# killerwhile/kafka-assignment-optimizer

Hardware: AMD Instinct MI355X
Metric: candidate assignments/sec (+ time_to_optimal_s), 10k-partition reassign (higher is better)
Workload: dtype int32

## Files before the change

### include/kao.h

```cpp
#ifndef KAO_H
#define KAO_H

#include <stdint.h>

#ifdef __cplusplus
extern "C" {
#endif

#define KAO_VERSION 103
#define KAO_NONE 0xFFFFu
#define KAO_MAX_RF 8
#define KAO_MAX_RACKS 255

enum {
    KAO_OK = 0,
    KAO_ERR_INVALID = -1,
    KAO_ERR_UNSUPPORTED = -2,
    KAO_ERR_NO_DEVICE = -3,
    KAO_ERR_HIP = -4,
    KAO_ERR_NOMEM = -5,
    KAO_ERR_NOT_INIT = -6
};

enum {
// ... 89 lines not shown
int kao_eval_plan_create(const kao_topic *t, kao_eval_plan **out);
int kao_eval_plan_run(kao_eval_plan *p, const void *d_candidates, int64_t n, void *d_objective ,
                      void *d_violations , void *d_best_key );
int kao_eval_plan_sync(kao_eval_plan *p, double *ms_last );
void kao_eval_plan_destroy(kao_eval_plan *p);

int kao_session_create(const kao_topic *topics, int32_t n_topics, const kao_opts *opts, kao_session **out);
int kao_session_step(kao_session *s);
int kao_session_sync(kao_session *s);
int kao_session_new_generation(kao_session *s);
int kao_session_best(kao_session *s, kao_result *results);
int kao_session_best_keys(kao_session *s, uint64_t *keys);
int kao_session_device_keys(kao_session *s, void **d_keys);
int kao_session_stats(kao_session *s, kao_stats *out);
int kao_session_small_launches(kao_session *s, int64_t *out);
int kao_session_chunked_launches(kao_session *s, int64_t *out);
int kao_search_chunk_plan(int32_t entries, int32_t resident, int32_t iters, int32_t forced, int32_t *out, int32_t cap);
int kao_session_bound_step(kao_session *s, const int64_t *target, int32_t iters);
int kao_session_set_prices(kao_session *s, int32_t topic, const int32_t *a, const int32_t *l, const int32_t *g);
int kao_session_adopt_prices(kao_session *s);
int kao_session_prices(kao_session *s, int32_t topic, int32_t *a, int32_t *l, int32_t *g);
int kao_session_bound_busy(kao_session *s);
int kao_session_bounds(kao_session *s, int64_t *upper_bound, int32_t *flags, int32_t *iters);
int kao_session_dual_state(kao_session *s, int32_t topic, int32_t *a, int32_t *l, int32_t *g, int64_t *best_dual);
int kao_session_set_dual_state(kao_session *s, int32_t topic, const int32_t *a, const int32_t *l, const int32_t *g);
int kao_lp_bound(const kao_topic *t, double tol, int32_t max_iters, int64_t *bound, int64_t *best_dual, int32_t *multipliers, double stats[8]);
int kao_lp_trace(const kao_topic *t, double tol, int32_t max_iters, double *trace, double stats[8], int32_t *multipliers);
int kao_lp_round(const kao_topic *t, double pert, uint32_t salt, double tol, int32_t max_iters, int32_t use_fallback, uint16_t *assignment,
                 int64_t *objective, int32_t violations[8], double stats[8]);
int kao_lp_round_host(const kao_topic *t, const uint8_t *q, const int32_t *zq, int32_t use_fallback, uint16_t *assignment, int32_t rep[4]);
int kao_dense_spd_test(const double *A, int32_t n, const double *rhs, double *factor, double *linv, double *x, double ms[2]);
int kao_search_band_row(int32_t lo, int32_t hi, int32_t c, int32_t force_plain, int32_t *fits);
int kao_search_rack_delta(int32_t lo, int32_t hi, int32_t c, int32_t dec);
int kao_lp_sharded_test(const kao_topic *t, const int32_t *devices, int32_t n_dev, double pert, uint32_t salt, double tol, int32_t max_iters,
                        int64_t *bound, uint16_t *assignment, int64_t *objective, int32_t violations[8], double stats[8]);
int kao_dual_bound(const kao_topic *t, int64_t target, int32_t iters, int32_t launches, int64_t *bound,
                   int64_t *best_dual, int32_t *iters_done, int32_t *flags, int32_t *multipliers);
int kao_session_restart_state(kao_session *s, int32_t topic, int32_t restart, uint16_t *final_state,
                              uint16_t *best_state, int32_t info[4]);
void kao_session_destroy(kao_session *s);

int kao_solve(const kao_topic *topics, int32_t n_topics, const kao_opts *opts, kao_result *results);
int kao_solve_multi(const kao_topic *topics, int32_t n_topics, const int32_t *devices, int32_t n_dev, const kao_opts *opts,
                    kao_result *results);
int kao_solve_capped(const kao_topic *topics, int32_t n_topics, const int32_t *replica_cap, const int32_t *devices, int32_t n_dev,
                     const kao_opts *opts, int32_t max_rounds, kao_result *results, int64_t *lagrangian_bound);
int kao_improve_cycles(const kao_topic *t, uint16_t *assignment, int32_t max_rounds, int64_t *objective, int32_t stats[8]);
int kao_cycle_matrices(const kao_topic *t, const uint16_t *assignment, int32_t layer, int32_t level, int32_t *dist, int32_t *mid,
                       uint32_t *slot);
int kao_cycle_square_plan(int32_t n, int32_t out[3]);
int kao_cycle_seeds(const kao_topic *t, const uint16_t *assignment, int32_t *table, int32_t *n_cfg);
int kao_cycle_pair_edges(const kao_topic *t, const uint16_t *assignment, int32_t gmin, int32_t *cost, int64_t stats[4]);

int kao_plan_waves(int32_t n_brokers, int32_t n_partitions, int32_t width, const uint16_t *current, const uint16_t *target,
                   int32_t max_per_broker, uint64_t seed, int32_t *wave , int32_t *n_waves, int32_t *lower_bound);

int kao_plan_waves_sized(int32_t n_brokers, int32_t n_partitions, int32_t width, const uint16_t *current, const uint16_t *target,
                         const uint64_t *size , uint64_t max_bytes_per_broker, int32_t max_per_broker,
                         uint64_t seed, int32_t *wave , int32_t *n_waves, int32_t *lower_bound);

int kao_balance_leaders(const kao_topic *t, uint16_t *assignment , int32_t *n_changed,
                        int64_t *objective ,
                        int32_t *status, int32_t stats[8] );

#define KAO_FAILOVER_MAX_BROKERS 8000
int kao_failover_order(int32_t n_brokers, int32_t n_racks, const uint8_t *rack_of ,
// ... 86 lines not shown
```

### kafka_assignment_optimizer_amd/_ffi.py

```python
from __future__ import annotations

import ctypes as C
import os

_HERE = os.path.dirname(os.path.abspath(__file__))
LIB_PATH = os.path.join(_HERE, "libkao.so")


class KaoTopic(C.Structure):
    _fields_ = [("n_brokers", C.c_int32), ("n_racks", C.c_int32), ("n_partitions", C.c_int32),
                ("rf", C.c_int32), ("rf_cur", C.c_int32),
                ("rack_of", C.POINTER(C.c_uint8)), ("current", C.POINTER(C.c_uint16)),
                ("w", (C.c_int32 * 2) * 2),
                ("rep_lo", C.c_int32), ("rep_hi", C.c_int32), ("lead_lo", C.c_int32), ("lead_hi", C.c_int32),
                ("rack_lo", C.c_int32), ("rack_hi", C.c_int32), ("prack_lo", C.c_int32), ("prack_hi", C.c_int32),
                ("broker_w", C.POINTER(C.c_int32)), ("broker_wl", C.POINTER(C.c_int32))]


class KaoOpts(C.Structure):
    _fields_ = [("seed", C.c_uint64), ("time_limit_s", C.c_double), ("restarts", C.c_int32),
                ("iters_per_launch", C.c_int32), ("max_launches", C.c_int32), ("obj_scale", C.c_int32),
                ("lam_min", C.c_int32), ("lam_max", C.c_int32), ("period_log2", C.c_int32),
                ("stop_at_bound", C.c_int32), ("profile", C.c_int32), ("dual_iters", C.c_int32),
                ("elite_period", C.c_int32), ("use_prices", C.c_int32), ("use_cycles", C.c_int32), ("islands", C.c_int32),
# ... 30 lines not shown
    "kao_evaluate": (C.c_int, [_P(KaoTopic), _P(C.c_uint16), _P(C.c_int64), _P(C.c_int32)]),
    "kao_evaluate_batch": (C.c_int, [_P(KaoTopic), _P(C.c_uint16), C.c_int64, _P(C.c_int32), _P(C.c_int32)]),
    "kao_eval_plan_create": (C.c_int, [_P(KaoTopic), _P(C.c_void_p)]),
    "kao_eval_plan_run": (C.c_int, [C.c_void_p, C.c_void_p, C.c_int64, C.c_void_p, C.c_void_p, C.c_void_p]),
    "kao_eval_plan_sync": (C.c_int, [C.c_void_p, _P(C.c_double)]),
    "kao_eval_plan_destroy": (None, [C.c_void_p]),
    "kao_session_create": (C.c_int, [_P(KaoTopic), C.c_int32, _P(KaoOpts), _P(C.c_void_p)]),
    "kao_session_step": (C.c_int, [C.c_void_p]),
    "kao_session_sync": (C.c_int, [C.c_void_p]),
    "kao_session_new_generation": (C.c_int, [C.c_void_p]),
    "kao_session_best": (C.c_int, [C.c_void_p, _P(KaoResult)]),
    "kao_session_best_keys": (C.c_int, [C.c_void_p, _P(C.c_uint64)]),
    "kao_session_device_keys": (C.c_int, [C.c_void_p, _P(C.c_void_p)]),
    "kao_session_stats": (C.c_int, [C.c_void_p, _P(KaoStats)]),
    "kao_session_small_launches": (C.c_int, [C.c_void_p, _P(C.c_int64)]),
    "kao_session_chunked_launches": (C.c_int, [C.c_void_p, _P(C.c_int64)]),
    "kao_search_chunk_plan": (C.c_int, [C.c_int32, C.c_int32, C.c_int32, C.c_int32, _P(C.c_int32), C.c_int32]),
    "kao_session_restart_state": (C.c_int, [C.c_void_p, C.c_int32, C.c_int32, _P(C.c_uint16), _P(C.c_uint16),
                                            _P(C.c_int32)]),
    "kao_session_bound_step": (C.c_int, [C.c_void_p, _P(C.c_int64), C.c_int32]),
    "kao_session_set_prices": (C.c_int, [C.c_void_p, C.c_int32, _P(C.c_int32), _P(C.c_int32), _P(C.c_int32)]),
    "kao_session_adopt_prices": (C.c_int, [C.c_void_p]),
    "kao_session_prices": (C.c_int, [C.c_void_p, C.c_int32, _P(C.c_int32), _P(C.c_int32), _P(C.c_int32)]),
    "kao_session_bound_busy": (C.c_int, [C.c_void_p]),
    "kao_session_bounds": (C.c_int, [C.c_void_p, _P(C.c_int64), _P(C.c_int32), _P(C.c_int32)]),
    "kao_session_dual_state": (C.c_int, [C.c_void_p, C.c_int32, _P(C.c_int32), _P(C.c_int32), _P(C.c_int32), _P(C.c_int64)]),
    "kao_session_set_dual_state": (C.c_int, [C.c_void_p, C.c_int32, _P(C.c_int32), _P(C.c_int32), _P(C.c_int32)]),
    "kao_lp_bound": (C.c_int, [_P(KaoTopic), C.c_double, C.c_int32, _P(C.c_int64), _P(C.c_int64), _P(C.c_int32), _P(C.c_double)]),
    "kao_lp_round": (C.c_int, [_P(KaoTopic), C.c_double, C.c_uint32, C.c_double, C.c_int32, C.c_int32, _P(C.c_uint16), _P(C.c_int64), _P(C.c_int32), _P(C.c_double)]),
    "kao_lp_round_host": (C.c_int, [_P(KaoTopic), _P(C.c_uint8), _P(C.c_int32), C.c_int32, _P(C.c_uint16), _P(C.c_int32)]),
    "kao_dense_spd_test": (C.c_int, [_P(C.c_double), C.c_int32, _P(C.c_double), _P(C.c_double), _P(C.c_double), _P(C.c_double), _P(C.c_double)]),
    "kao_search_band_row": (C.c_int, [C.c_int32, C.c_int32, C.c_int32, C.c_int32, _P(C.c_int32)]),
    "kao_search_rack_delta": (C.c_int, [C.c_int32, C.c_int32, C.c_int32, C.c_int32]),
    "kao_lp_sharded_test": (C.c_int, [_P(KaoTopic), _P(C.c_int32), C.c_int32, C.c_double, C.c_uint32, C.c_double, C.c_int32, _P(C.c_int64), _P(C.c_uint16),
                                      _P(C.c_int64), _P(C.c_int32), _P(C.c_double)]),
    "kao_lp_trace": (C.c_int, [_P(KaoTopic), C.c_double, C.c_int32, _P(C.c_double), _P(C.c_double), _P(C.c_int32)]),
    "kao_dual_bound": (C.c_int, [_P(KaoTopic), C.c_int64, C.c_int32, C.c_int32, _P(C.c_int64), _P(C.c_int64), _P(C.c_int32),
                                 _P(C.c_int32), _P(C.c_int32)]),
    "kao_session_destroy": (None, [C.c_void_p]),
    "kao_solve": (C.c_int, [_P(KaoTopic), C.c_int32, _P(KaoOpts), _P(KaoResult)]),
    "kao_solve_multi": (C.c_int, [_P(KaoTopic), C.c_int32, _P(C.c_int32), C.c_int32, _P(KaoOpts), _P(KaoResult)]),
    "kao_solve_capped": (C.c_int, [_P(KaoTopic), C.c_int32, _P(C.c_int32), _P(C.c_int32), C.c_int32, _P(KaoOpts), C.c_int32,
                                  _P(KaoResult), _P(C.c_int64)]),
    "kao_rccl_selftest": (C.c_int, [_P(C.c_int32), C.c_int32]),
    "kao_rccl_loopback_counts": (C.c_int, [_P(C.c_uint64)]),
    "kao_improve_cycles": (C.c_int, [_P(KaoTopic), _P(C.c_uint16), C.c_int32, _P(C.c_int64), _P(C.c_int32)]),
    "kao_cycle_matrices": (C.c_int, [_P(KaoTopic), _P(C.c_uint16), C.c_int32, C.c_int32, _P(C.c_int32), _P(C.c_int32), _P(C.c_uint32)]),
    "kao_cycle_square_plan": (C.c_int, [C.c_int32, _P(C.c_int32)]),
    "kao_cycle_seeds": (C.c_int, [_P(KaoTopic), _P(C.c_uint16), _P(C.c_int32), _P(C.c_int32)]),
    "kao_cycle_pair_edges": (C.c_int, [_P(KaoTopic), _P(C.c_uint16), C.c_int32, _P(C.c_int32), _P(C.c_int64)]),
    "kao_plan_waves": (C.c_int, [C.c_int32, C.c_int32, C.c_int32, _P(C.c_uint16), _P(C.c_uint16), C.c_int32, C.c_uint64,
                                 _P(C.c_int32), _P(C.c_int32), _P(C.c_int32)]),
    "kao_plan_waves_sized": (C.c_int, [C.c_int32, C.c_int32, C.c_int32, _P(C.c_uint16), _P(C.c_uint16), _P(C.c_uint64), C.c_uint64,
                                       C.c_int32, C.c_uint64, _P(C.c_int32), _P(C.c_int32), _P(C.c_int32)]),
    "kao_balance_leaders": (C.c_int, [_P(KaoTopic), _P(C.c_uint16), _P(C.c_int32), _P(C.c_int64), _P(C.c_int32), _P(C.c_int32)]),
    "kao_failover_order": (C.c_int, [C.c_int32, C.c_int32, _P(C.c_uint8), C.c_int32, C.c_int32, _P(C.c_uint16), C.c_int32, C.c_int32,
                                     _P(C.c_int32), _P(C.c_int32), _P(C.c_int32)]),
    "kao_balance_leaders_cluster": (C.c_int, [C.c_int32, C.c_int32, C.c_int32, _P(C.c_uint16), _P(C.c_int32), C.c_int32, _P(C.c_int32),
                                              _P(C.c_int32), C.c_int32, C.c_int32, C.c_int32, _P(C.c_int32), _P(C.c_int32), _P(C.c_int32),
                                              _P(C.c_int32), _P(C.c_int32)]),
    "kao_balance_leaders_weighted": (C.c_int, [C.c_int32, C.c_int32, C.c_int32, _P(C.c_uint16), _P(C.c_uint64), C.c_uint64, C.c_int32, C.c_int32,
                                               _P(C.c_int32), _P(C.c_uint64), _P(C.c_uint64), _P(C.c_uint64), _P(C.c_int32), _P(C.c_int64)]),
    "kao_wleaders_test_path": (C.c_int, [C.c_int32]),
    "kao_failover_order_weighted": (C.c_int, [C.c_int32, C.c_int32, _P(C.c_uint8), C.c_int32, C.c_int32, _P(C.c_uint16), _P(C.c_uint64), C.c_int32,
                                              C.c_uint64, C.c_int32, C.c_int32, _P(C.c_uint64), _P(C.c_int32), _P(C.c_int32), _P(C.c_int64)]),
    "kao_balance_disk": (C.c_int, [C.c_int32, C.c_int32, _P(C.c_uint8), C.c_int32, C.c_int32, _P(C.c_uint16), _P(C.c_uint64), C.c_int32, C.c_int32,
# ... 42 lines not shown
```

### kafka_assignment_optimizer_amd/csrc/kao_search.hip

```cpp
#include "kao_search_dev.h"

#include <map>
#include <mutex>
#include <tuple>

namespace kao {

struct SearchPiece {
    uint32_t entry;
    int32_t init, elite;
    uint32_t first, n;
    bool later;
    uint32_t ticket;
};
__device__ __forceinline__ void chunk_pass(uint32_t ticket);
template <class T> __device__ __forceinline__ T late_kernarg(size_t off) {
    auto p = (const __attribute__((address_space(4))) unsigned char *)__builtin_amdgcn_kernarg_segment_ptr();
    asm volatile("" : "+s"(p));
    return *reinterpret_cast<const __attribute__((address_space(4))) T *>(p + off);
}
static_assert(sizeof(SearchPools) % alignof(SearchParams) == 0, "late_kernarg: SearchParams follows SearchPools without padding");
constexpr size_t kArgPrm = sizeof(SearchPools);
__device__ __forceinline__ int4 sched_record(const int4 *sched, uint32_t ticket) {
    auto p = (const __attribute__((address_space(4))) int *)sched + 4 * (size_t)ticket;
// ... 193 lines not shown
        if (pc.later) rng = pl.chunk_rng[(size_t)g * 64 + lane];
        pl.chunk_rng[(size_t)g * 64 + lane] = pc.ticket;
    }

    const int plog = TD->period_log2 + (rho & 3);
    const uint32_t pmask = (1u << plog) - 1u;
    const uint32_t lrange = (uint32_t)(prm.lam_max - prm.lam_min + 1);
    const uint32_t RF8 = (uint32_t)T.RF << 8, R8 = (uint32_t)T.R << 8, m8 = (uint32_t)T.m << 8;

    const int T_tour = min(64, max(4, (T.P * T.RF) >> 2));
    uint32_t tour_off = lane < T_tour ? 0u : kKeyNull;
    asm volatile("" : "+v"(tour_off));
    const int GA = min(16, max(1, (T.P * T.RF) >> 8));
    const int x_rounds_full = (T.P + 63) >> 6;
    const bool x_windowed = x_rounds_full > 8;

    int lam_lo = prm.lam_min, lam_hi = prm.lam_max;
    uint32_t n_iters = kChunked ? pc.n : prm.iters, it_base = prm.launch * prm.iters + (kChunked ? pc.first : 0u);
    constexpr uint32_t kLpScanTwo = 1u << 29;
    uint32_t loop_pack = TD->P * TD->RF <= prm.scan2_max ? kLpScanTwo : 0u;
    if (kSmall) loop_pack |= ((uint32_t)prm.lam_min & 0xFFFu) | (((uint32_t)prm.lam_max & 0xFFFu) << 12) | (((uint32_t)plog & 31u) << 24);
    {
        uint32_t v0 = (uint32_t)lam_lo, v1 = (uint32_t)lam_hi, v2 = n_iters, v3 = it_base, v4 = loop_pack;
        asm volatile("" : "+v"(v2), "+v"(v3), "+v"(v4));
        if constexpr (!kSmall) {
            asm volatile("" : "+v"(v0), "+v"(v1));
            lam_lo = (int)__builtin_amdgcn_readfirstlane(v0); lam_hi = (int)__builtin_amdgcn_readfirstlane(v1);
        }
        n_iters = __builtin_amdgcn_readfirstlane(v2); it_base = __builtin_amdgcn_readfirstlane(v3);
        loop_pack = __builtin_amdgcn_readfirstlane(v4);
    }
    auto loop_flag = [&](uint32_t bit) { uint32_t lp = loop_pack; asm volatile("" : "+s"(lp)); return (lp & bit) != 0u; };
    constexpr bool kFuse = !kGlobalA && !kTeam && !kPriced;
    const bool fuse_ok = kFuse && T.Bx <= 16384;
    uint32_t jmp_a = 1u, jmp_c = 0u;
    if (fuse_ok)
        for (int n = (T.Bx + 63) >> 6; n > 0; --n) { jmp_a = (jmp_a * 0x6D2B79u) & 0xFFFFFFu; jmp_c = (jmp_c * 0x6D2B79u + 0x3C6EF3u) & 0xFFFFFFu; }
    best_obj = __builtin_amdgcn_readfirstlane(best_obj);
    for (uint32_t i = 0; i < n_iters; ++i) {
        const uint32_t it = it_base + i;
        const int type = (int)((0x1210u >> ((it & 7u) * 2u)) & 3u);
        int lam;
        if constexpr (kSmall) {
            uint32_t lp = loop_pack;
            asm volatile("" : "+s"(lp));
            const uint32_t plg = (lp >> 24) & 31u;
            const int lo_ = (int)(lp & 0xFFFu), hi_ = (int)((lp >> 12) & 0xFFFu);
            const uint32_t ph = it & ((1u << plg) - 1u);
            lam = best_obj < 0 ? hi_ : min(hi_, lo_ + (int)((2u * ph * (uint32_t)(hi_ - lo_ + 1)) >> plg));
        } else {
            const uint32_t ph = it & pmask;
            lam = best_obj < 0 ? lam_hi : min(lam_hi, lam_lo + (int)((2u * ph * lrange) >> plog));
        }
        const bool sampled = (type == 2) || (type == 0 && ((it >> 3) & 1u));

        auto finish = [&](auto ty, auto uni, uint32_t kmin, int win, int p, int k, int q, int j, uint32_t uw, uint32_t vw, int dV, int dObj) {
            constexpr int TY = decltype(ty)::value;
            auto of_win = [&](int v) { return decltype(uni)::value ? v : __builtin_amdgcn_readlane(v, win); };
            if (!kTeam) {
                if (kmin == kKeyNull) return;
                if ((int)(kmin >> 8) - kDBias > 0) return;
            }
            bool mine = true;
            int *rec = TR + ((i & 1u) * 16 + (uint32_t)wave) * kTeamRec;
            if (kTeam) {
                const bool ok = kmin != kKeyNull && (int)(kmin >> 8) - kDBias <= 0;
                if (lane == win) {
                    const uint32_t ro_ = uw >> 16, rn_ = vw >> 16;
                    const bool racks = ok && TY == 0 && ro_ != rn_;
                    rec[0] = ok ? 1 : 0; rec[1] = p; rec[2] = TY == 1 ? q : p;
                    rec[3] = (int)(uw & 0xFFFFu); rec[4] = (int)(vw & 0xFFFFu);
                    rec[5] = racks ? (int)ro_ : 0xFFFF; rec[6] = racks ? (int)rn_ : 0xFFFF;
                    rec[7] = dV; rec[8] = dObj;
                }
                __syncthreads();
                bool clash = false;
                if (lane < wave) {
                    const int *o = TR + ((i & 1u) * 16 + (uint32_t)lane) * kTeamRec;
                    if (o[0]) {
                        const int mp = rec[1], mq = rec[2], mb0 = rec[3], mb1 = rec[4], mr0 = rec[5], mr1 = rec[6];
                        clash = (o[1] == mp) | (o[1] == mq) | (o[2] == mp) | (o[2] == mq) | (o[3] == mb0) | (o[3] == mb1) | (o[4] == mb0) | (o[4] == mb1);
                        if (o[5] != 0xFFFF && mr0 != 0xFFFF) clash |= (o[5] == mr0) | (o[5] == mr1) | (o[6] == mr0) | (o[6] == mr1);
                    }
                }
                mine = ok && __ballot(clash) == 0ull;
            }

            constexpr bool kOneTrip = !kTeam && kSmall;
// ... 89 lines not shown
                        L.W[xx] = (uint16_t)wx;
                    }
                }
            }
            }
            if (kGlobalA) __builtin_amdgcn_fence(__ATOMIC_SEQ_CST, "workgroup");
            if (kTeam) {
                if (lane == 0) rec[9] = mine ? 1 : 0;
                __syncthreads();
                int dVs = 0, dOs = 0, na = 0;
                if (lane < n_waves) {
                    const int *o = TR + ((i & 1u) * 16 + (uint32_t)lane) * kTeamRec;
                    if (o[9]) { dVs = o[7]; dOs = o[8]; na = 1; }
                }
                V += wave_sum(dVs);
                obj += wave_sum(dOs);
                accepted += wave_sum(na);
            } else {
                V += of_win(dV);
                obj += of_win(dObj);
                accepted++;
            }
        };
        constexpr std::integral_constant<int, 0> kReplace{};
        constexpr std::integral_constant<int, 1> kExchange{};
        constexpr std::integral_constant<int, 2> kLeaderSwap{};

        if (sampled) {
            const int p = (int)rnd24_wide(rng, (uint32_t)T.P);
            const Part<NW> a = L.A[p];
            const Part<NW> c = CUR[p];
            uint32_t key = kKeyNull, vw = 0;
            int dV = 0, dObj = 0;
            if (type == 0) {
                const int k = (int)rnd24(rng, RF8);
                const uint32_t uw = sel_slot<NS>(a, k);
                const uint32_t ro = uw >> 16;
                const bool lead = k == 0;
                const uint32_t lw = lead ? 2u : 0u;
                const int wl = lead ? T.w00 : T.w01, wf = lead ? T.w10 : T.w11;
                const int g_old = role_w2<NS>(c, uw, wl, wf) + (hbw ? bw_of(BW[uw & 0xFFFFu], lead) : 0);
                const uint32_t wo = L.W[uw & 0xFFFFu];
                const int dV_old = wfld(wo, kWDecR) + wfldw(wo, kWDecL, lw);
                const int dV_rack_old = ddec(L.K[ro], T.rack_lo, T.rack_hi) + c7_delta(T.c7_dec, cnt4x2<NS>(a, ro));
                const int rsz_ro = RSZ[ro];
                int dP_old = 0, dP_rack_old = 0;
                if (kPriced) {
                    const uint32_t pro = PR[uw & 0xFFFFu];
                    dP_old = -(wflag(wo, kWPoutR) & price_rep(pro));
                    if (lead) dP_old -= wflag(wo, kWPoutL) & price_lead(pro);
                    dP_rack_old = p_out(L.K[ro], T.rack_lo, T.rack_hi, PG[ro]);
                }
                const int base_s = kSmall ? mad24s(S, g_old, kDBias) : 0;
#pragma unroll
                for (int g = 0; g < 4; ++g) {
                    uint32_t r, jj;
                    bool okg;
                    if (g < 2) {
                        r = rnd24(rng, R8);
                        jj = rnd24(rng, m8);
                        okg = (int)jj < RSZ[r];
                    } else {
                        r = ro;
                        jj = rnd24(rng, (uint32_t)rsz_ro << 8);
                        okg = true;
                    }
                    const uint32_t x = __umul24(r, (uint32_t)T.m) + jj;
// ... 162 lines not shown
#pragma unroll
                for (int s2 = 0; s2 < 2; ++s2) {
                    const int wA = s2 == 0 ? wA1 : wA2;
                    ps[s2] = __builtin_amdgcn_readlane(pl_, wA);
                    ks[s2] = __builtin_amdgcn_readlane(kl_, wA);
                    us[s2] = (uint32_t)__builtin_amdgcn_readlane((int)oldw_l, wA);
                    gs[s2] = __builtin_amdgcn_readlane(g_old_l, wA);
                    dvos[s2] = __builtin_amdgcn_readlane(dvo_l, wA);
                    v_rk[s2] = __builtin_amdgcn_readlane(dvr_l, wA);
                }
                const Part<NW> a1 = L.A[ps[0]], c1 = CUR[ps[0]], a2 = L.A[ps[1]], c2 = CUR[ps[1]];
                const uint32_t ro1 = us[0] >> 16, ro2 = us[1] >> 16;
                for (int r = lane; r < T.R; r += 64) {
                    const int dk = dinc(L.K[r], T.rack_lo, T.rack_hi);
                    const int v1 = ((uint32_t)r != ro1) ? v_rk[0] + dk + c7_delta(T.c7_inc, cnt4x2<NS>(a1, (uint32_t)r)) : 0;
                    const int v2 = ((uint32_t)r != ro2) ? v_rk[1] + dk + c7_delta(T.c7_inc, cnt4x2<NS>(a2, (uint32_t)r)) : 0;
                    L.RT[r] = kSmall ? (int)(((uint32_t)v2 & 0xFFFFu) | ((uint32_t)v1 << 16)) : (int)(((uint32_t)v1 & 0xFFFFu) | ((uint32_t)v2 << 16));
                }
                int lane_v = lane;
                asm volatile("" : "+v"(lane_v));
                const int li = lane_v & (NW - 1);
                const bool l2 = lane_v >= NW;
                const int p_l = l2 ? ps[1] : ps[0];
                const uint32_t ai = reinterpret_cast<const uint32_t *>(&L.A[p_l])[li], ci = reinterpret_cast<const uint32_t *>(&CUR[p_l])[li];
                const bool holds = (lane_v < 2 * NW) & (ai != kNoneW);
                uint32_t w_keep = 0;
                if (holds) w_keep = L.W[ai & 0xFFFFu];
                if (holds & !l2) L.W[ai & 0xFFFFu] = (uint16_t)(w_keep | kWNoCand);
                if (holds & l2) L.W[ai & 0xFFFFu] = (uint16_t)(L.W[ai & 0xFFFFu] | kWNoCand2);
                const bool hc = (lane_v < 2 * NW) & (ci != kNoneW);
                uint32_t w_ci = 0;
                if (hc) w_ci = L.W[ci & 0xFFFFu];
                const bool hm_l = hc & ((w_ci & (l2 ? kWNoCand2 : kWNoCand)) == 0u);
                const int mr_l = hm_l ? (int)((ci & 0xFFFFu) >> 6) : -1;
                int mr[2 * NW];
#pragma unroll
                for (int i2 = 0; i2 < 2 * NW; ++i2) mr[i2] = (i2 & (NW - 1)) < NS ? __builtin_amdgcn_readlane(mr_l, i2) : -1;
                const bool lead1 = ks[0] == 0, lead2 = ks[1] == 0;
                const uint32_t lw1 = lead1 ? 2u : 0u, lw2 = lead2 ? 2u : 0u;
                const int wl1 = lead1 ? T.w00 : T.w01, wf1 = lead1 ? T.w10 : T.w11, wl2 = lead2 ? T.w00 : T.w01, wf2 = lead2 ? T.w10 : T.w11;
                const int K01 = __mul24(S, gs[0]) + kDBias + __mul24(lam, dvos[0]);
                const int K02 = __mul24(S, gs[1]) + kDBias + __mul24(lam, dvos[1]);
                const uint32_t leadp = (lead2 ? 1u : 0u) | (lead1 ? 0x10000u : 0u);
                const uint32_t K0p = ((uint32_t)K02 & 0xFFFFu) | ((uint32_t)K01 << 16);
                const int wl1h = (int)((uint32_t)(S * wl1) << 16), wf1h = (int)((uint32_t)(S * wf1) << 16);
                const int wl2s = (int)((uint32_t)(S * wl2) & 0xFFFFu), wf2s = (int)((uint32_t)(S * wf2) & 0xFFFFu);
                uint32_t jc = jmp_c;
                asm volatile("" : "+v"(jc));
                uint32_t best1 = kKeyNull, best2 = kKeyNull;
                const short *Ws = reinterpret_cast<const short *>(L.W);
                auto scan_round2 = [&](auto with_w, int base, int rd, int w, int rt, uint32_t &key1, uint32_t &key2) {
                    const uint32_t st1 = lcg24(rng);
                    uint32_t st2;
                    asm("v_mad_u32_u24 %0, %1, %2, %3" : "=v"(st2) : "v"(st1), "s"(jmp_a), "v"(jc));
                    const int inc = wfld(w, kWIncR);
                    if constexpr (kSmall) {
                        uint32_t d = pk_mad_ss(pk_add(pk_mad_lo((uint32_t)wfld(w, kWIncL), leadp, (uint32_t)inc), (uint32_t)rt), (uint32_t)lam, K0p);
                        if (decltype(with_w)::value) {
                            const uint32_t x = (uint32_t)(base + lane);
                            const uint32_t xw = x | ((uint32_t)XR[x] << 16);
                            auto mask_of = [](bool b) { uint32_t m = b ? ~0u : 0u; asm("" : "+v"(m)); return m; };
                            const bool l1 = c1.w[0] == xw, l2 = c2.w[0] == xw;
                            bool f1 = false, f2 = false;
#pragma unroll
                            for (int i2 = 1; i2 < NS; ++i2) { f1 |= c1.w[i2] == xw; f2 |= c2.w[i2] == xw; }
                            auto and_or = [](uint32_t m, uint32_t w, uint32_t acc) { uint32_t r; asm("v_and_or_b32 %0, %1, %2, %3" : "=v"(r) : "v"(m), "s"(w), "v"(acc)); return r; };
                            uint32_t ws = mask_of(l1) & (uint32_t)wl1h;
                            ws = and_or(mask_of(f1), (uint32_t)wf1h, ws);
                            ws = and_or(mask_of(l2), (uint32_t)wl2s, ws);
                            ws = and_or(mask_of(f2), (uint32_t)wf2s, ws);
                            d = pk_sub(d, ws);
                        }
                        key1 = ((d | (uint32_t)w) & 0xFFFF0000u) | (st1 & 0xFF00u) | (uint32_t)rd;
                        key2 = ((d | (uint32_t)wflag(w, 14)) << 16) | (st2 & 0xFF00u) | (uint32_t)rd;
                        return;
                    }
                    int d1 = __mul24(lam, inc + wfldw(w, kWIncL, lw1) + wfldw(rt, 0, 16u)) + K01;
                    int d2 = __mul24(lam, inc + wfldw(w, kWIncL, lw2) + (rt >> 16)) + K02;
                    if (decltype(with_w)::value) {
                        const uint32_t x = (uint32_t)(base + lane);
                        const uint32_t xw = x | ((uint32_t)XR[x] << 16);
                        d1 -= __mul24(S, role_w2<NS>(c1, xw, wl1, wf1));
                        d2 -= __mul24(S, role_w2<NS>(c2, xw, wl2, wf2));
                    }
                    d1 = min(max(d1, 0), 2 * kDBias - 2);
                    d2 = min(max(d2, 0), 2 * kDBias - 2) | wflag(w, 14);
                    key1 = ((uint32_t)d1 << 16) | (st1 & 0xFF00u) | (uint32_t)rd | ((uint32_t)w & 0xFFFF0000u);
                    key2 = ((uint32_t)d2 << 16) | (st2 & 0xFF00u) | (uint32_t)rd;
                };
                const int n_rd = (T.Bx + 63) >> 6;
                int rd = 0, base = 0;
                while (rd < n_rd) {
                    int nxt = n_rd;
#pragma unroll
                    for (int i2 = 0; i2 < 2 * NW; ++i2)
                        if (mr[i2] >= rd) nxt = min(nxt, mr[i2]);
                    uint32_t k1a, k2a, k1b, k2b;
                    for (; rd + 1 < nxt; rd += 2, base += 128) {
                        const int wa = Ws[base + lane], wb = Ws[base + 64 + lane];
                        const uint32_t ra = XR[base + lane], rb = XR[base + 64 + lane];
                        const int rta = L.RT[ra], rtb = L.RT[rb];
                        scan_round2(std::false_type{}, base, rd, wa, rta, k1a, k2a);
                        scan_round2(std::false_type{}, base + 64, rd + 1, wb, rtb, k1b, k2b);
                        best1 = min(best1, min(k1a, k1b));
                        best2 = min(best2, min(k2a, k2b));
                    }
                    if (rd < nxt) { const int wa = Ws[base + lane]; scan_round2(std::false_type{}, base, rd, wa, L.RT[XR[base + lane]], k1a, k2a); best1 = min(best1, k1a); best2 = min(best2, k2a); ++rd; base += 64; }
                    if (rd < n_rd) { const int wa = Ws[base + lane]; scan_round2(std::true_type{}, base, rd, wa, L.RT[XR[base + lane]], k1a, k2a); best1 = min(best1, k1a); best2 = min(best2, k2a); ++rd; base += 64; }
                }
                asm("v_mad_u32_u24 %0, %0, %1, %2" : "+v"(rng) : "s"(jmp_a), "v"(jc));
                if (holds) L.W[ai & 0xFFFFu] = (uint16_t)w_keep;
                const uint32_t kw = wave_umin(min(((best1 >> 1) & ~127u) | (uint32_t)lane, ((best2 >> 1) & ~127u) | 64u | (uint32_t)lane));
                const bool two = (kw & 64u) != 0u;
                const uint32_t kmin = kw >> 7;
                const int win = (int)(kw & 63u);
                const int p = two ? ps[1] : ps[0], k = two ? ks[1] : ks[0];
                const uint32_t uw = two ? us[1] : us[0];
                if ((int)(kmin >> 8) - kDBias <= 0) {
                    const bool lead = k == 0;
                    const uint32_t bw_ = (uint32_t)__builtin_amdgcn_readlane((int)(two ? best2 : best1), win);
                    const uint32_t xs = ((bw_ & 255u) << 6) + (uint32_t)win;
                    const uint32_t rs = XR[xs];
                    const uint32_t ws = L.W[xs];
                    const int rts = L.RT[rs];
                    const uint32_t vw = xs | (rs << 16);
                    const int dV = wfld(ws, kWIncR) + wfldw(ws, kWIncL, lead ? 2u : 0u) + (two ? dvos[1] : dvos[0]) + ((two != kSmall) ? (rts >> 16) : wfldw(rts, 0, 16u));
                    int mx1 = -1, mx2 = -1;
#pragma unroll
                    for (int i2 = 0; i2 < NW; ++i2) { mx1 = max(mx1, mr[i2]); mx2 = max(mx2, mr[NW + i2]); }
                    const bool has_missing = (two ? mx2 : mx1) >= 0;
                    const int dObj = -(two ? gs[1] : gs[0]) + (has_missing ? (two ? role_w2<NS>(c2, vw, wl2, wf2) : role_w2<NS>(c1, vw, wl1, wf1)) : 0);
                    finish(kReplace, std::true_type{}, kmin, win, p, k, 0, 0, uw, vw, dV, dObj);
                }
            } else {
            auto slot_of = [&](int wA, int &p, int &k, uint32_t &uw, int &g_old, int &dV_old, int &dV_rack_old, Part<NW> &a, Part<NW> &c) {
                p = __builtin_amdgcn_readlane(pl_, wA);
                k = __builtin_amdgcn_readlane(kl_, wA);
                uw = (uint32_t)__builtin_amdgcn_readlane((int)oldw_l, wA);
                g_old = __builtin_amdgcn_readlane(g_old_l, wA);
                dV_old = __builtin_amdgcn_readlane(dvo_l, wA);
                dV_rack_old = __builtin_amdgcn_readlane(dvr_l, wA);
                if constexpr (kGlobalA) {
#pragma unroll
                    for (int i2 = 0; i2 < NW; ++i2) { a.w[i2] = (uint32_t)__builtin_amdgcn_readlane((int)a_l.w[i2], wA); c.w[i2] = (uint32_t)__builtin_amdgcn_readlane((int)c_l.w[i2], wA); }
                } else {
                    a = L.A[p];
                    c = CUR[p];
                }
            };
            if (type == 0) {
            uint32_t b_kmin = kKeyNull, b_uw = 0, b_vw = 0;
            int b_win = 0, b_p = 0, b_k = 0, b_dV = 0, b_dObj = 0;
#pragma nounroll
            for (int si = 0; si < (wA2 >= 0 ? 2 : 1); ++si) {
                int p, k, g_old, dV_old, dV_rack_old;
                uint32_t uw;
                Part<NW> a, c;
                slot_of(si == 0 ? wA1 : wA2, p, k, uw, g_old, dV_old, dV_rack_old, a, c);
                const bool lead = k == 0;
                const uint32_t ro = uw >> 16;
                uint32_t vw = 0;
                int dV = 0, dObj = 0;
                {
// ... 549 lines not shown
        const void *fn = reinterpret_cast<const void *>(decltype(k)::value);
        const auto key = std::make_tuple(fn, 64 * waves, lds, dev);
        std::lock_guard<std::mutex> lock(mu);
        const auto it = known.find(key);
        if (it != known.end()) { n = it->second; return; }
        if (hipOccupancyMaxActiveBlocksPerMultiprocessor(&n, fn, 64 * waves, lds) != hipSuccess) { (void)hipGetLastError(); n = 0; return; }
        known[key] = n;
    });
    return n;
}

bool launch_init(const SearchPools &pools, const SearchParams &prm, int n_blocks, int per_block, bool priced, int nw, int waves, void *stream) {
    const size_t lds = init_lds_bytes(prm.maxBx, prm.maxR, priced, prm.bw != 0);
    if (lds > 160 * 1024) return false;
    waves = waves > 0 ? std::min(kInitWaves, waves) : std::min(8, std::max(1, (prm.maxBx + 63) / 64));
    while (waves & (waves - 1)) waves &= waves - 1;
    const dim3 grid((unsigned)(n_blocks * per_block)), block((unsigned)(64 * waves));
    with_flags(priced, nw == 8, [&](auto p, auto k8) {
        launch_lds<k_init<decltype(p)::value, decltype(k8)::value ? 8 : 4>>(grid, block, lds, static_cast<hipStream_t>(stream), pools, prm, per_block);
    });
    return true;
}

}

extern "C" int kao_search_band_row(int32_t lo, int32_t hi, int32_t c, int32_t force_plain, int32_t *fits) {
    using namespace kao;
    const bool tab = band_tab_fits(lo, hi);
    if (fits) *fits = tab ? 1 : 0;
    if (tab && !force_plain) return (int)band_lookup_plain(c, band_tab_bias(lo), band_tab(lo, hi));
    const int a = std::min(std::max(c - lo, -1), 1), b = std::min(std::max(c - hi, -1), 1);
    return (int)((kBandTab >> (uint32_t)(6 * (3 * a + b) + 24)) & 63u);
}
extern "C" int kao_search_rack_delta(int32_t lo, int32_t hi, int32_t c, int32_t dec) {
    const uint32_t tab = kao::c7_tab(dec != 0, lo, hi);
    const uint32_t f = (tab >> ((2u * (uint32_t)c) & 31u)) & 3u;
    return (int)(f ^ 2u) - 2;
}
```

### kafka_assignment_optimizer_amd/csrc/kao_search_dev.h

```cpp
#pragma once
#include <hip/hip_runtime.h>

#include <type_traits>

#include "kao_device.h"
#include "kao_internal.h"

namespace kao {

__device__ __forceinline__ uint32_t fmix32(uint32_t h) {
    h ^= h >> 16; h *= 0x85EBCA6Bu; h ^= h >> 13; h *= 0xC2B2AE35u; h ^= h >> 16;
    return h;
}
__device__ __forceinline__ uint32_t xs32(uint32_t &s) {
    s ^= s << 13; s ^= s >> 17; s ^= s << 5;
    return s;
}
__device__ __forceinline__ uint32_t mulhi(uint32_t a, uint32_t b) { return __umulhi(a, b); }
__device__ __forceinline__ int band(int c, int lo, int hi) { return max(c - hi, 0) + max(lo - c, 0); }
__device__ __forceinline__ int dinc(int c, int lo, int hi) { return (int)(c >= hi) - (int)(c < lo); }
__device__ __forceinline__ int ddec(int c, int lo, int hi) { return (int)(c <= lo) - (int)(c > hi); }

template <int NW> struct alignas(16) Part { uint32_t w[NW]; };
__device__ __forceinline__ uint32_t sel4(const Part<4> &a, int k) {
// ... 204 lines not shown
}
constexpr int kBandTabLast = 4;
constexpr bool band_tab_fits(int lo, int hi) { return lo >= 0 && lo <= hi && hi <= 0xFFFF && hi - lo + 2 <= kBandTabLast; }
constexpr uint32_t band_tab(int lo, int hi) {
    uint32_t t = 0;
    for (int i = 0; i <= kBandTabLast; ++i) {
        const int c = lo - 1 + (i < hi - lo + 2 ? i : hi - lo + 2);
        const int a = c < lo ? -1 : (c > lo ? 1 : 0), b = c < hi ? -1 : (c > hi ? 1 : 0);
        t |= (uint32_t)band_entry_of(a, b) << (6 * i);
    }
    return t;
}
constexpr int band_tab_bias(int lo) { return 6 - 6 * lo; }
constexpr uint32_t band_lookup_plain(int c, int bias, uint32_t tab) {
    const int x = 6 * c + bias;
    return (tab >> (x < 0 ? 0 : (x > 6 * kBandTabLast ? 6 * kBandTabLast : x))) & 63u;
}
__device__ __forceinline__ uint32_t band_lookup(int c, int bias, uint32_t tab) {
    int x;
    asm("v_mad_i32_i24 %0, %1, 6, %2\n\tv_med3_i32 %0, %0, 0, 24" : "=&v"(x) : "v"(c), "v"(bias));
    static_assert(6 * kBandTabLast == 24, "the clamp's inline constant");
    return __builtin_amdgcn_ubfe(tab, (uint32_t)x, 6u);
}
template <bool kTab> __device__ __forceinline__ uint32_t band_row(int c, int r0, int r1) {
    if constexpr (kTab) return band_lookup(c, r0, (uint32_t)r1);
    else return band_entry(c, r0, r1);
}
__device__ __forceinline__ uint32_t band_fields(const TopicRegs &T, uint32_t c) {
    return band_entry((int)(c & 0xFFFFu), T.rep_lo, T.rep_hi) | (band_entry((int)(c >> 16), T.lead_lo, T.lead_hi) << 6);
}
constexpr uint32_t kWRowR = 0x003Fu, kWRowL = 0x0FC0u;
constexpr uint32_t kWNoCand = 0x8000u;
constexpr uint32_t kWNoCand2 = 0x4000u;
template <int NW> __device__ __forceinline__ void rebuild_band_state(const TopicRegs &T, const WaveLds<NW> &L, const uint8_t *XR, uint32_t inv, int lane, int stride = 64) {
    for (int x = lane; x < ((T.Bx + 63) & ~63); x += stride) L.W[x] = (uint16_t)(XR[x] == inv ? (kWNoCand | kWNoCand2) : band_fields(T, L.C[x]));
}

struct FillTabs {
    uint16_t *W;
    const uint8_t *XR;
    const int *K;
    int *RT;
    const uint32_t *PR;
    const int *PG;
    const uint32_t *BW;
};
constexpr uint32_t kFillTieStep = 0x165667B1u;
template <int NS, int NW> __device__ __forceinline__ void fill_mark(uint16_t *W, const Part<NW> &a, int lane) {
    const uint32_t ai = sel_slot<NS>(a, lane & (NW - 1));
    if ((lane < NS) & (ai != kNoneW)) W[ai & 0xFFFFu] |= (uint16_t)kWNoCand;
}
template <int NS, int NW> __device__ __forceinline__ void fill_unmark(uint16_t *W, const Part<NW> &a, int lane) {
    const uint32_t ai = sel_slot<NS>(a, lane & (NW - 1));
    if ((lane < NS) & (ai != kNoneW)) W[ai & 0xFFFFu] &= (uint16_t)~kWNoCand;
}
template <int NS, bool kPriced, int NW> __device__ __forceinline__ void fill_rack_table(const TopicRegs &T, const FillTabs &F, const Part<NW> &a, int lane) {
    for (int r = lane; r < T.R; r += 64) {
        const int kr = F.K[r];
        int v = dinc(kr, T.rack_lo, T.rack_hi) + c7_delta(T.c7_inc, cnt4x2<NS>(a, (uint32_t)r));
        if (kPriced) v = (v & 0xFF) | (p_in(kr, T.rack_lo, T.rack_hi, F.PG[r]) * 256);
        F.RT[r] = v;
    }
}
template <int NS, bool kPriced, bool kClamp, bool kWithW, int NW>
__device__ __forceinline__ uint32_t fill_round_on(const TopicRegs &T, const FillTabs &F, const Part<NW> &c, int x, int rd, uint32_t h, int lam, int S, bool lead, int w, uint32_t r, int rt) {
    const uint32_t lw = lead ? 2u : 0u, lf = lead ? 1u : 0u;
// ... 128 lines not shown
```

Before: 962.1 billion.

## Use ballot bitmask for missing-round scan and rebalance move-type schedule

In the small-topic search kernel, the per-slot readlane array of missing-candidate rounds is replaced by a ballot over slot lanes and a 64-bit round bitmask, with the next round found by count-trailing-zeros. The bitmask is coarsened for larger broker counts. This cuts per-round scalar min loops and register use. The unpriced path also gets a new 16-entry move-type schedule, which shifts how often each move kind runs and so changes search behaviour and quality, not just speed. A host test entry point for the mask scan is added.

```diff
diff --git a/include/kao.h b/include/kao.h
--- a/include/kao.h
+++ b/include/kao.h
@@ -145,6 +145,7 @@
 int kao_dense_spd_test(const double *A, int32_t n, const double *rhs, double *factor, double *linv, double *x, double ms[2]);
 int kao_search_band_row(int32_t lo, int32_t hi, int32_t c, int32_t force_plain, int32_t *fits);
 int kao_search_rack_delta(int32_t lo, int32_t hi, int32_t c, int32_t dec);
+int kao_search_scan_next(const int32_t *rounds, int32_t n, int32_t rd, int32_t n_rd);
 int kao_lp_sharded_test(const kao_topic *t, const int32_t *devices, int32_t n_dev, double pert, uint32_t salt, double tol, int32_t max_iters,
                         int64_t *bound, uint16_t *assignment, int64_t *objective, int32_t violations[8], double stats[8]);
 int kao_dual_bound(const kao_topic *t, int64_t target, int32_t iters, int32_t launches, int64_t *bound,
diff --git a/kafka_assignment_optimizer_amd/_ffi.py b/kafka_assignment_optimizer_amd/_ffi.py
--- a/kafka_assignment_optimizer_amd/_ffi.py
+++ b/kafka_assignment_optimizer_amd/_ffi.py
@@ -86,6 +86,7 @@
     "kao_dense_spd_test": (C.c_int, [_P(C.c_double), C.c_int32, _P(C.c_double), _P(C.c_double), _P(C.c_double), _P(C.c_double), _P(C.c_double)]),
     "kao_search_band_row": (C.c_int, [C.c_int32, C.c_int32, C.c_int32, C.c_int32, _P(C.c_int32)]),
     "kao_search_rack_delta": (C.c_int, [C.c_int32, C.c_int32, C.c_int32, C.c_int32]),
+    "kao_search_scan_next": (C.c_int, [_P(C.c_int32), C.c_int32, C.c_int32, C.c_int32]),
     "kao_lp_sharded_test": (C.c_int, [_P(KaoTopic), _P(C.c_int32), C.c_int32, C.c_double, C.c_uint32, C.c_double, C.c_int32, _P(C.c_int64), _P(C.c_uint16),
                                       _P(C.c_int64), _P(C.c_int32), _P(C.c_double)]),
     "kao_lp_trace": (C.c_int, [_P(KaoTopic), C.c_double, C.c_int32, _P(C.c_double), _P(C.c_double), _P(C.c_int32)]),
diff --git a/kafka_assignment_optimizer_amd/csrc/kao_search.hip b/kafka_assignment_optimizer_amd/csrc/kao_search.hip
--- a/kafka_assignment_optimizer_amd/csrc/kao_search.hip
+++ b/kafka_assignment_optimizer_amd/csrc/kao_search.hip
@@ -249,6 +249,7 @@
     }
     auto loop_flag = [&](uint32_t bit) { uint32_t lp = loop_pack; asm volatile("" : "+s"(lp)); return (lp & bit) != 0u; };
     constexpr bool kFuse = !kGlobalA && !kTeam && !kPriced;
+    constexpr bool kScanMask = kSmall;
     const bool fuse_ok = kFuse && T.Bx <= 16384;
     uint32_t jmp_a = 1u, jmp_c = 0u;
     if (fuse_ok)
@@ -256,7 +257,17 @@
     best_obj = __builtin_amdgcn_readfirstlane(best_obj);
     for (uint32_t i = 0; i < n_iters; ++i) {
         const uint32_t it = it_base + i;
-        const int type = (int)((0x1210u >> ((it & 7u) * 2u)) & 3u);
+        uint32_t kind = 0u;
+        int type;
+        bool sampled;
+        if constexpr (kPriced) {
+            type = (int)((0x1210u >> ((it & 7u) * 2u)) & 3u);
+            sampled = (type == 2) || (type == 0 && ((it >> 3) & 1u));
+        } else {
+            kind = (0xDEDF1210u >> ((it & 15u) * 2u)) & 3u;
+            sampled = kind >= 2u;
+            type = (int)kind;
+        }
         int lam;
         if constexpr (kSmall) {
             uint32_t lp = loop_pack;
@@ -269,8 +280,6 @@
             const uint32_t ph = it & pmask;
             lam = best_obj < 0 ? lam_hi : min(lam_hi, lam_lo + (int)((2u * ph * lrange) >> plog));
         }
-        const bool sampled = (type == 2) || (type == 0 && ((it >> 3) & 1u));
-
         auto finish = [&](auto ty, auto uni, uint32_t kmin, int win, int p, int k, int q, int j, uint32_t uw, uint32_t vw, int dV, int dObj) {
             constexpr int TY = decltype(ty)::value;
             auto of_win = [&](int v) { return decltype(uni)::value ? v : __builtin_amdgcn_readlane(v, win); };
@@ -426,7 +435,7 @@
             const Part<NW> c = CUR[p];
             uint32_t key = kKeyNull, vw = 0;
             int dV = 0, dObj = 0;
-            if (type == 0) {
+            if (kPriced ? type == 0 : kind == 3u) {
                 const int k = (int)rnd24(rng, RF8);
                 const uint32_t uw = sel_slot<NS>(a, k);
                 const uint32_t ro = uw >> 16;
@@ -655,10 +664,31 @@
                 uint32_t w_ci = 0;
                 if (hc) w_ci = L.W[ci & 0xFFFFu];
                 const bool hm_l = hc & ((w_ci & (l2 ? kWNoCand2 : kWNoCand)) == 0u);
-                const int mr_l = hm_l ? (int)((ci & 0xFFFFu) >> 6) : -1;
-                int mr[2 * NW];
-#pragma unroll
-                for (int i2 = 0; i2 < 2 * NW; ++i2) mr[i2] = (i2 & (NW - 1)) < NS ? __builtin_amdgcn_readlane(mr_l, i2) : -1;
+                const int n_rd = (T.Bx + 63) >> 6;
+                constexpr uint32_t kSlotLanes = ((1u << NS) - 1u) * ((1u << NW) + 1u);
+                uint32_t hm_b = 0u;
+                unsigned long long wmask = 0ull;
+                int mr[2 * NW] = {};
+                if constexpr (kScanMask) {
+                    hm_b = (uint32_t)__ballot(hm_l) & kSlotLanes;
+                    const int rd_l = (int)((ci & 0xFFFFu) >> 6);
+                    for (uint32_t b = hm_b; b != 0u; b &= b - 1u)
+                        wmask |= 1ull << (uint32_t)(__builtin_amdgcn_readlane(rd_l, __builtin_ctz(b)) >> scan_mask_shift(n_rd));
+                } else {
+                    const int mr_l = hm_l ? (int)((ci & 0xFFFFu) >> 6) : -1;
+#pragma unroll
+                    for (int i2 = 0; i2 < 2 * NW; ++i2) mr[i2] = (i2 & (NW - 1)) < NS ? __builtin_amdgcn_readlane(mr_l, i2) : -1;
+                }
+                auto scan_next = [&](int rd) {
+                    if constexpr (kScanMask) return scan_next_mask(wmask, rd, n_rd, scan_mask_shift(n_rd));
+                    else {
+                        int nxt = n_rd;
+#pragma unroll
+                        for (int i2 = 0; i2 < 2 * NW; ++i2)
+                            if (mr[i2] >= rd) nxt = min(nxt, mr[i2]);
+                        return nxt;
+                    }
+                };
                 const bool lead1 = ks[0] == 0, lead2 = ks[1] == 0;
                 const uint32_t lw1 = lead1 ? 2u : 0u, lw2 = lead2 ? 2u : 0u;
                 const int wl1 = lead1 ? T.w00 : T.w01, wf1 = lead1 ? T.w10 : T.w11, wl2 = lead2 ? T.w00 : T.w01, wf2 = lead2 ? T.w10 : T.w11;
@@ -711,13 +741,9 @@
                     key1 = ((uint32_t)d1 << 16) | (st1 & 0xFF00u) | (uint32_t)rd | ((uint32_t)w & 0xFFFF0000u);
                     key2 = ((uint32_t)d2 << 16) | (st2 & 0xFF00u) | (uint32_t)rd;
                 };
-                const int n_rd = (T.Bx + 63) >> 6;
                 int rd = 0, base = 0;
                 while (rd < n_rd) {
-                    int nxt = n_rd;
-#pragma unroll
-                    for (int i2 = 0; i2 < 2 * NW; ++i2)
-                        if (mr[i2] >= rd) nxt = min(nxt, mr[i2]);
+                    const int nxt = scan_next(rd);
                     uint32_t k1a, k2a, k1b, k2b;
                     for (; rd + 1 < nxt; rd += 2, base += 128) {
                         const int wa = Ws[base + lane], wb = Ws[base + 64 + lane];
@@ -748,10 +774,14 @@
                     const int rts = L.RT[rs];
                     const uint32_t vw = xs | (rs << 16);
                     const int dV = wfld(ws, kWIncR) + wfldw(ws, kWIncL, lead ? 2u : 0u) + (two ? dvos[1] : dvos[0]) + ((two != kSmall) ? (rts >> 16) : wfldw(rts, 0, 16u));
-                    int mx1 = -1, mx2 = -1;
-#pragma unroll
-                    for (int i2 = 0; i2 < NW; ++i2) { mx1 = max(mx1, mr[i2]); mx2 = max(mx2, mr[NW + i2]); }
-                    const bool has_missing = (two ? mx2 : mx1) >= 0;
+                    bool has_missing;
+                    if constexpr (kScanMask) has_missing = (hm_b & (two ? ((1u << NW) - 1u) << NW : (1u << NW) - 1u)) != 0u;
+                    else {
+                        int mx1 = -1, mx2 = -1;
+#pragma unroll
+                        for (int i2 = 0; i2 < NW; ++i2) { mx1 = max(mx1, mr[i2]); mx2 = max(mx2, mr[NW + i2]); }
+                        has_missing = (two ? mx2 : mx1) >= 0;
+                    }
                     const int dObj = -(two ? gs[1] : gs[0]) + (has_missing ? (two ? role_w2<NS>(c2, vw, wl2, wf2) : role_w2<NS>(c1, vw, wl1, wf1)) : 0);
                     finish(kReplace, std::true_type{}, kmin, win, p, k, 0, 0, uw, vw, dV, dObj);
                 }
@@ -1367,6 +1397,14 @@
     const int a = std::min(std::max(c - lo, -1), 1), b = std::min(std::max(c - hi, -1), 1);
     return (int)((kBandTab >> (uint32_t)(6 * (3 * a + b) + 24)) & 63u);
 }
+extern "C" int kao_search_scan_next(const int32_t *rounds, int32_t n, int32_t rd, int32_t n_rd) {
+    using namespace kao;
+    if (!rounds || n < 0 || rd < 0 || rd >= n_rd || n_rd > 256) return -1;
+    unsigned long long wmask = 0ull;
+    for (int i = 0; i < n; ++i)
+        if (rounds[i] >= 0 && rounds[i] < n_rd) wmask |= 1ull << (uint32_t)(rounds[i] >> scan_mask_shift(n_rd));
+    return scan_next_mask(wmask, rd, n_rd, scan_mask_shift(n_rd));
+}
 extern "C" int kao_search_rack_delta(int32_t lo, int32_t hi, int32_t c, int32_t dec) {
     const uint32_t tab = kao::c7_tab(dec != 0, lo, hi);
     const uint32_t f = (tab >> ((2u * (uint32_t)c) & 31u)) & 3u;
diff --git a/kafka_assignment_optimizer_amd/csrc/kao_search_dev.h b/kafka_assignment_optimizer_amd/csrc/kao_search_dev.h
--- a/kafka_assignment_optimizer_amd/csrc/kao_search_dev.h
+++ b/kafka_assignment_optimizer_amd/csrc/kao_search_dev.h
@@ -260,6 +260,13 @@
 constexpr uint32_t kWRowR = 0x003Fu, kWRowL = 0x0FC0u;
 constexpr uint32_t kWNoCand = 0x8000u;
 constexpr uint32_t kWNoCand2 = 0x4000u;
+constexpr int scan_mask_shift(int n_rd) { return n_rd <= 64 ? 0 : (n_rd <= 128 ? 1 : 2); }
+constexpr int scan_next_mask(unsigned long long wmask, int rd, int n_rd, int shift) {
+    const unsigned long long m = wmask >> (uint32_t)(rd >> shift);
+    if (!m) return n_rd;
+    const int g = ((rd >> shift) + (int)__builtin_ctzll(m)) << shift;
+    return g > rd ? g : rd;
+}
 template <int NW> __device__ __forceinline__ void rebuild_band_state(const TopicRegs &T, const WaveLds<NW> &L, const uint8_t *XR, uint32_t inv, int lane, int stride = 64) {
     for (int x = lane; x < ((T.Bx + 63) & ~63); x += stride) L.W[x] = (uint16_t)(XR[x] == inv ? (kWNoCand | kWNoCand2) : band_fields(T, L.C[x]));
 }
```

After: 996.6 billion (median of 6 runs). 3.6% higher.
